# hengdashi/cuda_gcn

Measured on AMD Instinct MI355X. Metric: epochs_per_sec, higher is better.
Workload: dtype f32

## Files before the change

cuda_gcn_amd/csrc/class_bf16x3.h:

```cpp
#pragma once
#include "dense_kernels.h"
#include "bf16x3_split.h"

struct ClsB3 { bf16x8 h, m, l; };

__device__ __forceinline__ ClsB3 cls_planes(const float v[8]) {
    BxPlanes P;
#pragma unroll
    for (int i = 0; i < 4; i++) bx_split2(v[2 * i], v[2 * i + 1], P.w[0][i], P.w[1][i], P.w[2][i]);
    return ClsB3{bx_plane(P, 0), bx_plane(P, 1), bx_plane(P, 2)};
}
__device__ __forceinline__ void cls_mac(f32x16 &c, const ClsB3 &A, const ClsB3 &B) {
    c = MFMA_BF16(A.l, B.h, c);
    c = MFMA_BF16(A.m, B.m, c);
    c = MFMA_BF16(A.h, B.l, c);
    c = MFMA_BF16(A.m, B.h, c);
    c = MFMA_BF16(A.h, B.m, c);
    c = MFMA_BF16(A.h, B.h, c);
}
__device__ __forceinline__ ClsB3 cls_lds(const uint4 *img, int piece, int lane) {
    const uint4 h = img[(piece * 3 + 0) * 64 + lane], m = img[(piece * 3 + 1) * 64 + lane], l = img[(piece * 3 + 2) * 64 + lane];
    return ClsB3{__builtin_bit_cast(bf16x8, h), __builtin_bit_cast(bf16x8, m), __builtin_bit_cast(bf16x8, l)};
}
__device__ __forceinline__ void cls_lds_put(uint4 *img, int piece, int lane, const float v[8]) {
    BxPlanes P;
#pragma unroll
    for (int i = 0; i < 4; i++) bx_split2(v[2 * i], v[2 * i + 1], P.w[0][i], P.w[1][i], P.w[2][i]);
#pragma unroll
    for (int pl = 0; pl < 3; pl++) img[(piece * 3 + pl) * 64 + lane] = make_uint4(P.w[pl][0], P.w[pl][1], P.w[pl][2], P.w[pl][3]);
}

struct ClsFwdArgs {
    const float *h1; int ldh;
    const float *w2; int ldw;
    float *z0; int ldz;
    int m, p, n_rb;
};
constexpr int CLS_FWD_LDS = 8 * 2 * 3 * 1024;

#define CLS_WAIT2(N, x, y) asm volatile("s_waitcnt vmcnt(" #N ")" : "+v"(x), "+v"(y) :: "memory")
template <int S>
__device__ __forceinline__ void cls_fwd_issue(f32x4 (&R)[16], uint32_t vo, u32x4 rs) {
    bx_bload16<64 * S>(R[2 * S], vo, rs);
    bx_bload16<64 * S + 16>(R[2 * S + 1], vo, rs);
}

#define CLS_TIE4(R, i) "+v"((R)[i]), "+v"((R)[(i) + 1]), "+v"((R)[(i) + 2]), "+v"((R)[(i) + 3])
#define CLS_WAIT_ALL16(R) asm volatile("s_waitcnt vmcnt(0)" : CLS_TIE4(R, 0), CLS_TIE4(R, 4), CLS_TIE4(R, 8), CLS_TIE4(R, 12) :: "memory")

__global__ __launch_bounds__(256) void class_fwd_bf16x3_kernel(ClsFwdArgs a) {
    extern __shared__ __attribute__((aligned(16))) uint4 cls_img[];
    const int lane = threadIdx.x & 63, wave = threadIdx.x >> 6, li = lane & 31, hh = lane >> 5;
    for (int idx = threadIdx.x; idx < 8 * 2 * 64; idx += 256) {
        const int ln = idx & 63, cb = (idx >> 6) & 1, s = idx >> 7;
        const int c = 32 * cb + (ln & 31), k0 = 16 * s + 8 * (ln >> 5);
        const bool ok = c < a.p;
        const float *wp = a.w2 + (size_t)k0 * a.ldw + (ok ? c : 0);
        float v[8];
#pragma unroll
        for (int j = 0; j < 8; j++) v[j] = wp[(size_t)j * a.ldw];
#pragma unroll
        for (int j = 0; j < 8; j++) v[j] = ok ? v[j] : 0.f;
        cls_lds_put(cls_img, s * 2 + cb, ln, v);
    }
    __syncthreads();
    const u32x4 rs_h = bx_make_rsrc(a.h1, (uint32_t)a.m * (uint32_t)a.ldh * 4u);
    const int stride = gridDim.x * 4;
    int rb = blockIdx.x * 4 + wave;
    auto voff = [&](int b) { return ((uint32_t)(b * 32 + li) * (uint32_t)a.ldh + 8u * hh) * 4u; };
    auto issue = [&](f32x4 (&Q)[16], uint32_t vo) __attribute__((always_inline)) {
        cls_fwd_issue<0>(Q, vo, rs_h); cls_fwd_issue<1>(Q, vo, rs_h); cls_fwd_issue<2>(Q, vo, rs_h); cls_fwd_issue<3>(Q, vo, rs_h);
        cls_fwd_issue<4>(Q, vo, rs_h); cls_fwd_issue<5>(Q, vo, rs_h); cls_fwd_issue<6>(Q, vo, rs_h); cls_fwd_issue<7>(Q, vo, rs_h);
    };
    f32x4 R[16];
    issue(R, voff(rb));
    for (; rb < a.n_rb; rb += stride) {
        const uint32_t vn = voff(rb + stride);
        f32x16 acc[2];
#pragma unroll
        for (int cb = 0; cb < 2; cb++)
#pragma unroll
            for (int r = 0; r < 16; r++) acc[cb][r] = 0.f;
#define CLS_FWD_STEP(S)                                                                                                      \
        {                                                                                                                    \
            CLS_WAIT2(14, R[2 * S], R[2 * S + 1]);                                                                           \
            const float v[8] = {R[2 * S][0], R[2 * S][1], R[2 * S][2], R[2 * S][3], R[2 * S + 1][0], R[2 * S + 1][1], R[2 * S + 1][2], R[2 * S + 1][3]}; \
            ClsB3 A = cls_planes(v);                                                                                         \
            asm volatile("" : "+v"(A.h), "+v"(A.m), "+v"(A.l));                \
            cls_fwd_issue<S>(R, vn, rs_h);                                                                                   \
            cls_mac(acc[0], A, cls_lds(cls_img, S * 2, lane));                                                               \
            if (a.p > 32) cls_mac(acc[1], A, cls_lds(cls_img, S * 2 + 1, lane));                                             \
        }
        CLS_FWD_STEP(0) CLS_FWD_STEP(1) CLS_FWD_STEP(2) CLS_FWD_STEP(3) CLS_FWD_STEP(4) CLS_FWD_STEP(5) CLS_FWD_STEP(6) CLS_FWD_STEP(7)
#undef CLS_FWD_STEP
#pragma unroll
        for (int cb = 0; cb < 2; cb++)
#pragma unroll
            for (int r = 0; r < 16; r++) {
                const int orow = rb * 32 + (r & 3) + 8 * (r >> 2) + 4 * hh, c = 32 * cb + li;
                if (orow < a.m && c < a.p) a.z0[(size_t)orow * a.ldz + c] = acc[cb][r];
            }
    }
    CLS_WAIT_ALL16(R);
}

struct ClsBwdArgs {
    const float *dz; int lddz;
    const float *h1; int ldh;
    const float *w2; int ldw;
    float *da; int ldda;
    const uint32_t *bits;
    const float *rowscale; float scale;
    float *slab; int p_ld;
    int m, p, n_rb;
};
constexpr int CLS_BWD_PAIRS = 4;
constexpr int CLS_BWD_IMG = 4 * 4 * 3 * 1024;
constexpr int CLS_BWD_LDS = CLS_BWD_IMG + 128 * 64 * 4;

struct ClsCol { float z[2][8], h[2][8]; };
#define CLS_TIE8(x) "+v"((x)[0]), "+v"((x)[1]), "+v"((x)[2]), "+v"((x)[3]), "+v"((x)[4]), "+v"((x)[5]), "+v"((x)[6]), "+v"((x)[7])
#define CLS_WAIT_COL(N, c) asm volatile("s_waitcnt vmcnt(%32)" : CLS_TIE8((c).z[0]), CLS_TIE8((c).z[1]), CLS_TIE8((c).h[0]), CLS_TIE8((c).h[1]) : "n"(N) : "memory")

template <int NKS>
__global__ __launch_bounds__(512) void class_bwd_bf16x3_kernel(ClsBwdArgs a) {
    extern __shared__ __attribute__((aligned(16))) uint4 cls_img[];
    float *red = reinterpret_cast<float *>(cls_img) + CLS_BWD_IMG / 4;
    const int lane = threadIdx.x & 63, wave = threadIdx.x >> 6, li = lane & 31, hh = lane >> 5;
    const int pair = wave >> 1, half = wave & 1;
    for (int idx = threadIdx.x; idx < NKS * 4 * 64; idx += 512) {
        const int ln = idx & 63, fb = (idx >> 6) & 3, s = idx >> 8;
        const int f = 32 * fb + (ln & 31), c0 = 16 * s + 8 * (ln >> 5);
        float v[8];
#pragma unroll
        for (int j = 0; j < 8; j++) v[j] = a.w2[(size_t)f * a.ldw + min(c0 + j, a.p - 1)];
#pragma unroll
        for (int j = 0; j < 8; j++) v[j] = c0 + j < a.p ? v[j] : 0.f;
        cls_lds_put(cls_img, s * 4 + fb, ln, v);
    }
    for (int i = threadIdx.x; i < 128 * 64; i += 512) red[i] = 0.f;
    __syncthreads();

    const u32x4 rs_z = bx_make_rsrc(a.dz, (uint32_t)a.m * (uint32_t)a.lddz * 4u);
    const u32x4 rs_h = bx_make_rsrc(a.h1, (uint32_t)a.m * (uint32_t)a.ldh * 4u);
    const u32x4 rs_b = bx_make_rsrc(a.bits, (uint32_t)a.m * 16u);
    const u32x4 rs_s = bx_make_rsrc(a.rowscale ? a.rowscale : a.dz, a.rowscale ? (uint32_t)a.m * 4u : 0u);
    uint32_t so_z[8], so_h[8];
#pragma unroll
    for (int j = 0; j < 8; j++) { so_z[j] = (uint32_t)j * (uint32_t)a.lddz * 4u; so_h[j] = (uint32_t)j * (uint32_t)a.ldh * 4u; }

    f32x4 Z[2 * NKS];
    f32x4 KB;
    float RSC;
    auto issue_l1 = [&](int b) __attribute__((always_inline)) {
        const uint32_t row = (uint32_t)(b * 32 + li);
        const uint32_t vz = (row * (uint32_t)a.lddz + 8u * hh) * 4u;
        bx_bload16<0>(Z[0], vz, rs_z); bx_bload16<16>(Z[1], vz, rs_z);
        if constexpr (NKS > 1) { bx_bload16<64>(Z[2], vz, rs_z); bx_bload16<80>(Z[3], vz, rs_z); }
        if constexpr (NKS > 2) { bx_bload16<128>(Z[4], vz, rs_z); bx_bload16<144>(Z[5], vz, rs_z); }
        if constexpr (NKS > 3) { bx_bload16<192>(Z[6], vz, rs_z); bx_bload16<208>(Z[7], vz, rs_z); }
        bx_bload16<0>(KB, row * 16u, rs_b); bx_bload4(RSC, row * 4u, rs_s, 0u);
    };
    constexpr int NL1 = 2 * NKS + 2;
    ClsCol Cc;
    auto issue_col = [&](int b, int s2) __attribute__((always_inline)) {
        const uint32_t r0 = (uint32_t)(b * 32 + 16 * s2 + 8 * hh);
#pragma unroll
        for (int cb = 0; cb < 2; cb++) {
            const uint32_t c = 32u * cb + li;
            const uint32_t vo = c < (uint32_t)a.lddz ? (r0 * (uint32_t)a.lddz + c) * 4u : 0xFFFFF000u;
#pragma unroll
            for (int j = 0; j < 8; j++) bx_bload4(Cc.z[cb][j], vo, rs_z, so_z[j]);
        }
#pragma unroll
        for (int f2 = 0; f2 < 2; f2++) {
            const uint32_t vo = (r0 * (uint32_t)a.ldh + 32u * (2 * half + f2) + li) * 4u;
#pragma unroll
            for (int j = 0; j < 8; j++) bx_bload4(Cc.h[f2][j], vo, rs_h, so_h[j]);
        }
    };

    f32x16 dw[2][2];
#pragma unroll
    for (int f2 = 0; f2 < 2; f2++)
#pragma unroll
        for (int cb = 0; cb < 2; cb++)
#pragma unroll
            for (int r = 0; r < 16; r++) dw[f2][cb][r] = 0.f;

    const int stride = gridDim.x * CLS_BWD_PAIRS;
    int rb = blockIdx.x * CLS_BWD_PAIRS + pair;
    issue_l1(rb);
    for (; rb < a.n_rb; rb += stride) {
        issue_col(rb, 0);
        asm volatile("s_waitcnt vmcnt(32)" : "+v"(KB), "+v"(RSC) :: "memory");
#pragma unroll
        for (int i = 0; i < 2 * NKS; i++) asm volatile("" : "+v"(Z[i]));
        const uint32_t kw[2] = {__float_as_uint(KB[2 * half]), __float_as_uint(KB[2 * half + 1])};
        const float sc = a.rowscale ? a.scale * RSC : a.scale;
        f32x16 acc[2];
#pragma unroll
        for (int f2 = 0; f2 < 2; f2++)
#pragma unroll
            for (int r = 0; r < 16; r++) acc[f2][r] = 0.f;
#pragma unroll
        for (int s = 0; s < NKS; s++) {
            float v[8] = {Z[2 * s][0], Z[2 * s][1], Z[2 * s][2], Z[2 * s][3], Z[2 * s + 1][0], Z[2 * s + 1][1], Z[2 * s + 1][2], Z[2 * s + 1][3]};
            const int c0 = 16 * s + 8 * hh;
#pragma unroll
            for (int j = 0; j < 8; j++) v[j] = c0 + j < a.p ? v[j] : 0.f;
            const ClsB3 B = cls_planes(v);
#pragma unroll
            for (int f2 = 0; f2 < 2; f2++) cls_mac(acc[f2], B, cls_lds(cls_img, s * 4 + 2 * half + f2, lane));
        }
#pragma unroll
        for (int r = 0; r < 16; r++) {
            const int rl = (r & 3) + 8 * (r >> 2) + 4 * hh, orow = rb * 32 + rl;
            const float scr = __shfl(sc, rl, WAVE);
            const uint32_t w0 = __shfl(kw[0], rl, WAVE), w1 = __shfl(kw[1], rl, WAVE);
            if (orow < a.m) {
                float *dp = a.da + (size_t)orow * a.ldda + 64 * half + li;
                dp[0] = ((w0 >> li) & 1u) ? acc[0][r] * scr : 0.f;
                dp[32] = ((w1 >> li) & 1u) ? acc[1][r] * scr : 0.f;
            }
        }
        issue_l1(rb + stride);
#pragma unroll
        for (int s2 = 0; s2 < 2; s2++) {
            if (s2 == 0) CLS_WAIT_COL(NL1, Cc);
            else CLS_WAIT_COL(0, Cc);
            ClsB3 Bz[2], Ah[2];
#pragma unroll
            for (int cb = 0; cb < 2; cb++) {
                float v[8];
#pragma unroll
                for (int j = 0; j < 8; j++) v[j] = (32 * cb + li < a.p) ? Cc.z[cb][j] : 0.f;
                Bz[cb] = cls_planes(v);
            }
#pragma unroll
            for (int f2 = 0; f2 < 2; f2++) Ah[f2] = cls_planes(Cc.h[f2]);
            if (s2 == 0) issue_col(rb, 1);
#pragma unroll
            for (int f2 = 0; f2 < 2; f2++) {
                cls_mac(dw[f2][0], Ah[f2], Bz[0]);
                if (a.p > 32) cls_mac(dw[f2][1], Ah[f2], Bz[1]);
            }
        }
        asm volatile("s_waitcnt vmcnt(0)" : "+v"(KB), "+v"(RSC) :: "memory");
#pragma unroll
        for (int i = 0; i < 2 * NKS; i++) asm volatile("" : "+v"(Z[i]));
    }
    asm volatile("s_waitcnt vmcnt(0)" : "+v"(KB), "+v"(RSC) :: "memory");
#pragma unroll
    for (int i = 0; i < 2 * NKS; i++) asm volatile("" : "+v"(Z[i]));
    for (int w = 0; w < CLS_BWD_PAIRS; w++) {
        if (pair == w) {
#pragma unroll
            for (int f2 = 0; f2 < 2; f2++)
#pragma unroll
                for (int cb = 0; cb < 2; cb++)
#pragma unroll
                    for (int r = 0; r < 16; r++) {
                        const int f = 32 * (2 * half + f2) + (r & 3) + 8 * (r >> 2) + 4 * hh;
                        red[f * 64 + 32 * cb + li] += dw[f2][cb][r];
                    }
        }
        __syncthreads();
    }
    float *slab = a.slab + (size_t)blockIdx.x * 128 * a.p_ld;
    for (int i = threadIdx.x; i < 128 * a.p_ld; i += 512) {
        const int f = i / a.p_ld, c = i % a.p_ld;
        slab[i] = c < 64 ? red[f * 64 + c] : 0.f;
    }
}

static inline bool cls_fwd_fits(const float *a, int lda, const float *c, int ldc, int m, int n, int p) {
    return n == 128 && p >= 1 && p <= 64 && m >= 2048 && lda % 4 == 0 && lda >= 128 && ldc % 4 == 0 && aligned16(a) && aligned16(c) &&
           (uint64_t)m * lda * 4 < (1ull << 32);
}
static inline bool cls_bwd_fits(const float *a, int lda, const float *dc, int lddc, const float *da, int ldda, const uint32_t *bits, int wpr,
                                int m, int n, int p) {
    return n == 128 && p >= 1 && p <= 64 && m >= 2048 && wpr == 4 && bits && aligned16(bits) && a && lda >= 128 && lddc % 4 == 0 &&
           lddc >= (p + 15) / 16 * 16 && ldda % 4 == 0 && ldda >= 128 && aligned16(dc) && aligned16(da) &&
           (uint64_t)m * lda * 4 < (1ull << 32) && (uint64_t)m * lddc * 4 < (1ull << 32);
}

static int launch_class_fwd(gcnhip_ctx *c, const float *a, int lda, const float *b, int ldb, float *z, int ldz, int m, int p) {
    ClsFwdArgs k;
    k.h1 = a; k.ldh = lda; k.w2 = b; k.ldw = ldb; k.z0 = z; k.ldz = ldz; k.m = m; k.p = p; k.n_rb = ceil_div(m, 32);
    int grid = ceil_div(k.n_rb, 4);
    if (grid > c->n_cu * 3) grid = c->n_cu * 3;
    class_fwd_bf16x3_kernel<<<grid, 256, CLS_FWD_LDS, c->stream>>>(k);
    GCNHIP_LAUNCH_CHECK();
    return 0;
}
```

cuda_gcn_amd/csrc/matmul.hip:

```cpp
#include "dense_kernels.h"
#include "class_bf16x3.h"

extern "C" {

int gcnhip_matmul_fwd(gcnhip_ctx *c, const float *a, int lda, const float *b, int ldb,
                      float *cc, int ldc, int m, int n, int p) {
    if (!c || !a || !b || !cc || m < 0 || n <= 0 || p <= 0 || lda < n || ldb < p || ldc < p) return -1;
    if (m == 0) return 0;
    if (c->opt.gemm_bf16x3 >= 1 && cls_fwd_fits(a, lda, cc, ldc, m, n, p)) return launch_class_fwd(c, a, lda, b, ldb, cc, ldc, m, p);
    return launch_rowstream(c, a, lda, b, ldb, 0, cc, ldc, m, n, p, nullptr, 0, 1.f);
}

static int launch_class_bwd(gcnhip_ctx *c, const float *a, int lda, const float *b, int ldb, const float *dc, int lddc, float *da, int ldda,
                            float *db, int lddb, int m, int p, float scale, const uint32_t *bits, const float *rowscale) {
    ClsBwdArgs k;
    k.dz = dc; k.lddz = lddc; k.h1 = a; k.ldh = lda; k.w2 = b; k.ldw = ldb; k.da = da; k.ldda = ldda; k.bits = bits;
    k.rowscale = rowscale; k.scale = scale; k.p_ld = (p + 3) / 4 * 4; k.m = m; k.p = p; k.n_rb = ceil_div(m, 32);
    const int nks = (p + 15) / 16;
    int grid = ceil_div(k.n_rb, CLS_BWD_PAIRS);
    if (grid > c->n_cu) grid = c->n_cu;
    const int rc = ensure_slab(c, (size_t)grid * 128 * k.p_ld * sizeof(float));
    if (rc) return rc;
    k.slab = c->slab;
#define CLS_BWD(NKS)                                                                                                              \
    do {                                                                                                                          \
        GCNHIP_TRY(hipFuncSetAttribute((const void *)class_bwd_bf16x3_kernel<NKS>, hipFuncAttributeMaxDynamicSharedMemorySize, CLS_BWD_LDS)); \
        class_bwd_bf16x3_kernel<NKS><<<grid, 512, CLS_BWD_LDS, c->stream>>>(k);                                                  \
    } while (0)
    switch (nks) {
        case 1: CLS_BWD(1); break;
        case 2: CLS_BWD(2); break;
        case 3: CLS_BWD(3); break;
        default: CLS_BWD(4); break;
    }
#undef CLS_BWD
    GCNHIP_LAUNCH_CHECK();
    launch_slab_reduce(k.slab, grid, 128, p, k.p_ld, db, lddb, c->stream);
    GCNHIP_LAUNCH_CHECK();
    return 0;
}

static int da_product(gcnhip_ctx *c, bool fits_only, const float *dc, int lddc, const float *b, int ldb, float *da, int ldda, int m, int n, int p,
                      const float *h, int ldh, float scale, const uint32_t *bits, int wpr, const float *rowscale) {
    if (fits_only) return rowstream_plan(dc, lddc, da, ldda, p, n, h, ldh, bits).fits ? 0 : -1;
    return launch_rowstream(c, dc, lddc, b, ldb, 1, da, ldda, m, p, n, h, ldh, scale, bits, wpr, rowscale);
}

static int matmul_bwd_impl(gcnhip_ctx *c, const float *a, int lda, const float *b, int ldb,
                           const float *dc, int lddc, float *da, int ldda, float *db, int lddb,
                           int m, int n, int p, int fused, float scale) {
    if (!c || !a || !b || !dc || m < 0 || n <= 0 || p <= 0 || lda < n || ldb < p || lddc < p) return -1;
    if ((da && ldda < n) || (db && lddb < p)) return -1;
    if (m == 0) {
        if (db) for (int j = 0; j < n; j++) GCNHIP_TRY(hipMemsetAsync(db + (size_t)j * lddb, 0, p * sizeof(float), c->stream));
        return 0;
    }
    auto da_call = [&](bool fits_only) { return da_product(c, fits_only, dc, lddc, b, ldb, da, ldda, m, n, p, fused ? a : nullptr, lda, scale, nullptr, 0, nullptr); };
    if (da && da_call(true)) return -1;
    if (db) {
        const int rc = launch_atb(c, a, lda, dc, lddc, db, lddb, m, n, p, 0, 0.f, 0, nullptr, 0, nullptr);
        if (rc) return rc;
    }
    return da ? da_call(false) : 0;
}

int gcnhip_matmul_bwd(gcnhip_ctx *c, const float *a, int lda, const float *b, int ldb,
                      const float *dc, int lddc, float *da, int ldda, float *db, int lddb,
                      int m, int n, int p) {
    return matmul_bwd_impl(c, a, lda, b, ldb, dc, lddc, da, ldda, db, lddb, m, n, p, 0, 1.f);
}

int gcnhip_matmul_bwd_fused(gcnhip_ctx *c, const float *a, int lda, const float *b, int ldb,
                            const float *dc, int lddc, float *da, int ldda, float *db, int lddb,
                            int m, int n, int p, float relu_dropout_scale) {
    return matmul_bwd_impl(c, a, lda, b, ldb, dc, lddc, da, ldda, db, lddb, m, n, p, 1, relu_dropout_scale);
}

int gcnhip_matmul_bwd_fused_bits(gcnhip_ctx *c, const float *a, int lda, const float *b, int ldb,
                                 const float *dc, int lddc, float *da, int ldda, float *db, int lddb,
                                 int m, int n, int p, float relu_dropout_scale, const uint32_t *pos_bits, int words_per_row) {
    if (!c || !a || !b || !dc || !da || !pos_bits || m < 0 || n <= 0 || p <= 0 || lda < n || ldb < p || lddc < p || ldda < n) return -1;
    if (db && lddb < p) return -1;
    if (words_per_row * 32 < n) return -1;
    if (m == 0) return matmul_bwd_impl(c, a, lda, b, ldb, dc, lddc, nullptr, 0, db, lddb, m, n, p, 0, 1.f);
    auto da_call = [&](bool fits_only) {
        return da_product(c, fits_only, dc, lddc, b, ldb, da, ldda, m, n, p, nullptr, 0, relu_dropout_scale, pos_bits, words_per_row, nullptr);
    };
    if (da_call(true)) return -1;
    if (db) {
        const int rc = launch_atb(c, a, lda, dc, lddc, db, lddb, m, n, p, 0, 0.f, 0, nullptr, 0, nullptr);
        if (rc) return rc;
    }
    return da_call(false);
}

int gcnhip_matmul_bwd_ex(gcnhip_ctx *c, const float *a, int lda, const float *b, int ldb,
                         const float *dc, int lddc, float *da, int ldda, float *db, int lddb,
                         int m, int n, int p, float relu_dropout_scale, const uint32_t *pos_bits, int words_per_row,
                         const float *d_da_row_scale) {
    if (!c || !b || !dc || !da || m < 0 || n <= 0 || p <= 0 || ldb < p || lddc < p || ldda < n) return -1;
    if ((db || !pos_bits) && (!a || lda < n)) return -1;
    if (db && lddb < p) return -1;
    if (pos_bits && words_per_row * 32 < n) return -1;
    if (!(relu_dropout_scale > 0.f)) return -1;
    if (m == 0) {
        if (db) for (int j = 0; j < n; j++) GCNHIP_TRY(hipMemsetAsync(db + (size_t)j * lddb, 0, p * sizeof(float), c->stream));
        return 0;
    }
    if (db && c->opt.gemm_bf16x3 >= 1 && cls_bwd_fits(a, lda, dc, lddc, da, ldda, pos_bits, words_per_row, m, n, p))
        return launch_class_bwd(c, a, lda, b, ldb, dc, lddc, da, ldda, db, lddb, m, p, relu_dropout_scale, pos_bits, d_da_row_scale);
// ... 25 lines not shown
```

cuda_gcn_amd/csrc/graphsum.hip:

```cpp
#include "dense_kernels.h"
#include <algorithm>
#include <stdlib.h>

struct GsArgs {
    const int *indptr, *indices;
    const float *coef;
    const int4 *tasks;
    int n_tasks, n_rows, nnz;
    size_t table_bytes;
    const float *in;
    const uint16_t *in_bf;
    float *out;
    float *partials;
    int ld_in, ld_out, part_ld, dim;
    int n_slices;
    int bounds[9];
    int fuse, training, thr;
    float scale;
    uint64_t seed, elem_offset;
    const uint32_t *d_epoch;
    const uint8_t *keep_mask;
    const uint32_t *row_bits;
    const uint32_t *out_bits;
    uint32_t *pos_bits;
// ... 45 lines not shown
#pragma unroll
        for (int i = 0; i < 4; i++) x[i] *= (bits >> i & 1u) ? a.scale : 0.f;
    }
    return make_float4(x[0], x[1], x[2], x[3]);
}

template <int L>
__device__ __forceinline__ void xent_row_epilogue4(const GsArgs &a, int row, float4 z, int lane, int l, int g, int col0) {
#pragma clang fp contract(off)
    const int t = a.xe_truth[row];
    const int nv4 = (a.dim + 3) >> 2;
    float *gr = a.xe_grad ? a.xe_grad + (size_t)row * a.xe_ld_grad : nullptr;
    if (t < 0) {
        if (a.xe_training && gr && g == 0 && l < nv4) *reinterpret_cast<float4 *>(gr + col0) = make_float4(0.f, 0.f, 0.f, 0.f);
        if (lane == 0) *reinterpret_cast<float2 *>(a.xe_terms + 2 * (size_t)row) = make_float2(0.f, 0.f);
        return;
    }
    float x[4] = {z.x, z.y, z.z, z.w};
    float mx = -1e30f;
#pragma unroll
    for (int i = 0; i < 4; i++) if (col0 + i < a.dim) mx = fmaxf(mx, x[i]);
#pragma unroll
    for (int m = 1; m < L; m <<= 1) mx = fmaxf(mx, __shfl_xor(mx, m, WAVE));
    mx = __int_as_float(__builtin_amdgcn_readfirstlane(__float_as_int(mx)));
    const int ti = t & 3;
    const float sel = ti == 0 ? x[0] : (ti == 1 ? x[1] : (ti == 2 ? x[2] : x[3]));
    const float tv = __int_as_float(__builtin_amdgcn_readlane(__float_as_int(sel), t >> 2));
    const bool correct = !(mx > tv);
    float ex[4];
#pragma unroll
    for (int i = 0; i < 4; i++) {
        x[i] -= mx;
        ex[i] = col0 + i < a.dim ? expf(x[i]) : 0.f;
    }
    float se = 0.f;
    for (int q = 0; q < nv4; q++) {
#pragma unroll
        for (int i = 0; i < 4; i++) se += __int_as_float(__builtin_amdgcn_readlane(__float_as_int(ex[i]), q));
    }
    const float term = logf(se) - (tv - mx);
    if (lane == 0) *reinterpret_cast<float2 *>(a.xe_terms + 2 * (size_t)row) = make_float2(term, correct ? 1.f : 0.f);
    if (a.xe_training && gr && g == 0 && l < nv4) {
        const float gs = a.xe_grad_scale ? a.xe_grad_scale[row] : 1.f;
        float o[4];
#pragma unroll
        for (int i = 0; i < 4; i++) {
            float p = ex[i] / se;
            if (col0 + i == t) p = (float)((double)p - 1.0);
            o[i] = col0 + i < a.dim ? (a.xe_grad_scale ? (p / a.xe_count) * gs : p / a.xe_count) : 0.f;
        }
        *reinterpret_cast<float4 *>(gr + col0) = make_float4(o[0], o[1], o[2], o[3]);
    }
}
__device__ __forceinline__ void xent_row_epilogue1(const GsArgs &a, int row, float v, int lane) {
#pragma clang fp contract(off)
    const int t = a.xe_truth[row];
    const int nv4 = (a.dim + 3) >> 2;
    float *gr = a.xe_grad ? a.xe_grad + (size_t)row * a.xe_ld_grad : nullptr;
    if (t < 0) {
        if (a.xe_training && gr && lane < 4 * nv4) gr[lane] = 0.f;
        if (lane == 0) *reinterpret_cast<float2 *>(a.xe_terms + 2 * (size_t)row) = make_float2(0.f, 0.f);
        return;
    }
    float mx = lane < a.dim ? fmaxf(-1e30f, v) : -1e30f;
#pragma unroll
    for (int m = 1; m < WAVE; m <<= 1) mx = fmaxf(mx, __shfl_xor(mx, m, WAVE));
    const float tv = __int_as_float(__builtin_amdgcn_readlane(__float_as_int(v), t));
    const bool correct = !(mx > tv);
    const float x = v - mx;
    const float ex = lane < a.dim ? expf(x) : 0.f;
    float se = 0.f;
    for (int j = 0; j < 4 * nv4; j++) se += __int_as_float(__builtin_amdgcn_readlane(__float_as_int(ex), j));
    const float term = logf(se) - (tv - mx);
    if (lane == 0) *reinterpret_cast<float2 *>(a.xe_terms + 2 * (size_t)row) = make_float2(term, correct ? 1.f : 0.f);
    if (a.xe_training && gr && lane < 4 * nv4) {
        float p = ex / se;
        if (lane == t) p = (float)((double)p - 1.0);
        const float gs = a.xe_grad_scale ? a.xe_grad_scale[row] : 1.f;
        gr[lane] = lane < a.dim ? (a.xe_grad_scale ? (p / a.xe_count) * gs : p / a.xe_count) : 0.f;
    }
}

constexpr int GS_U = 4;
template <int L, int GS_U>
__device__ __forceinline__ float4 gather_chunk(const GsArgs &a, const float *in, int my_idx, float my_c, int cnt, int g, float4 acc) {
    constexpr int G = WAVE / L;
    const int iters = (cnt + G - 1) / G;
    int k = 0;
    if (!a.row_bits) {
        for (; (k + GS_U) * G <= cnt; k += GS_U) {
            float4 v[GS_U];
            float cc[GS_U];
#pragma unroll
            for (int u = 0; u < GS_U; u++) {
                const int src = (k + u) * G + g;
                const int j = __shfl(my_idx, src, WAVE);
                cc[u] = __shfl(my_c, src, WAVE);
                v[u] = *reinterpret_cast<const float4 *>(in + (size_t)j * a.ld_in);
            }
#pragma unroll
            for (int u = 0; u < GS_U; u++) acc = f4_fma(cc[u], v[u], acc);
        }
    }
    const int j_safe = __shfl(my_idx, 0, WAVE);
    for (; k < iters; k += GS_U) {
        float4 v[GS_U];
        float cc[GS_U];
        bool on[GS_U];
#pragma unroll
        for (int u = 0; u < GS_U; u++) {
            const int src = (k + u) * G + g;
            const int j = __shfl(my_idx, src & 63, WAVE);
            cc[u] = __shfl(my_c, src & 63, WAVE);
            on[u] = src < cnt && cc[u] != 0.f;
            v[u] = *reinterpret_cast<const float4 *>(in + (size_t)(on[u] ? j : j_safe) * a.ld_in);
        }
#pragma unroll
        for (int u = 0; u < GS_U; u++) {
            const float4 n = f4_fma(cc[u], v[u], acc);
            acc.x = on[u] ? n.x : acc.x; acc.y = on[u] ? n.y : acc.y; acc.z = on[u] ? n.z : acc.z; acc.w = on[u] ? n.w : acc.w;
        }
    }
    return acc;
}


struct GsTask { int row, e0, e1, slot; };
__device__ __forceinline__ GsTask gs_task(const GsArgs &a, int t) {
    if (a.n_tasks) {
        const int4 tk = a.tasks[t];
        return {tk.x, tk.y, tk.z, tk.w};
    }
    return {t, a.indptr[t], a.indptr[t + 1], -1};
}

template <bool SLICED>
__device__ __forceinline__ bool gs_block_task(const GsArgs &a, int &t, int &cslice) {
    const int xcd = blockIdx.x & 7, q = blockIdx.x >> 3;
    cslice = SLICED ? xcd % a.n_slices : blockIdx.y;
    const int g_id = SLICED ? xcd / a.n_slices : xcd;
    t = a.bounds[g_id] + q * (blockDim.x >> 6) + (threadIdx.x >> 6);
    return t < a.bounds[g_id + 1];
}

__device__ __forceinline__ void gs_load_edges(const GsArgs &a, int base, int cnt, int lane, int &my_idx, float &my_c) {
    my_idx = 0;
    my_c = 0.f;
    if (lane < cnt) {
        my_idx = a.indices[base + lane];
        my_c = a.coef ? a.coef[base + lane] : 1.f;
        if (a.row_bits && !((a.row_bits[my_idx >> 5] >> (my_idx & 31)) & 1u)) my_c = 0.f;
    }
}

template <int L>
__device__ __forceinline__ float4 gs_group_sum(float4 acc) {
#pragma unroll
    for (int m = L; m < WAVE; m <<= 1) acc = f4_add(acc, f4_shfl_xor(acc, m));
    return acc;
}

__device__ __forceinline__ void gs_store_partial(const GsArgs &a, int slot, int col0, float4 acc) {
    *reinterpret_cast<float4 *>(a.partials + (size_t)slot * a.part_ld + col0) = acc;
}
__device__ __forceinline__ void gs_store_partial(const GsArgs &a, int slot, int col0, float4 lo, float4 hi) {
    gs_store_partial(a, slot, col0, lo);
    gs_store_partial(a, slot, col0 + 4, hi);
}

__device__ __forceinline__ float gs_segment_sum(const GsArgs &a, int first, int ns, int col, float v) {
    const float *pp = a.partials + (size_t)first * a.part_ld + col;
    int k = 0;
    for (; k + 4 <= ns; k += 4) {
        const float p0 = pp[(size_t)k * a.part_ld], p1 = pp[(size_t)(k + 1) * a.part_ld];
        const float p2 = pp[(size_t)(k + 2) * a.part_ld], p3 = pp[(size_t)(k + 3) * a.part_ld];
        v += p0; v += p1; v += p2; v += p3;
    }
    const float p0 = pp[(size_t)min(k, ns - 1) * a.part_ld], p1 = pp[(size_t)min(k + 1, ns - 1) * a.part_ld];
    const float p2 = pp[(size_t)min(k + 2, ns - 1) * a.part_ld];
    if (k < ns) v += p0;
    if (k + 1 < ns) v += p1;
    if (k + 2 < ns) v += p2;
    return v;
}

__device__ __forceinline__ float4 gs_post4(const GsArgs &a, int row, float4 acc) {
    if (a.post) { const float ps = a.post[row]; acc.x *= ps; acc.y *= ps; acc.z *= ps; acc.w *= ps; }
    return acc;
}
__device__ __forceinline__ void gs_store_row4(const GsArgs &a, float *o, int col0, float4 acc) {
    if (col0 + 4 <= a.dim) {
        *reinterpret_cast<float4 *>(o) = acc;
    } else {
        const float x[4] = {acc.x, acc.y, acc.z, acc.w};
        for (int i = 0; col0 + i < a.dim; i++) o[i] = x[i];
    }
}

template <int L, int U = GS_U, bool SLICED = false>
__global__ __launch_bounds__(256) void graphsum_vec_kernel(GsArgs a) {
    const int lane = threadIdx.x & 63;
    int t, cslice;
    if (!gs_block_task<SLICED>(a, t, cslice)) return;
    const auto [row, e0, e1, slot] = gs_task(a, t);
    if (!row_wanted(a, row)) return;
    const int g = lane / L, l = lane % L;
    const int col0 = (cslice * L + l) * 4;
    const bool active = col0 < a.dim;
    const float *in = a.in + (active ? col0 : 0);
    float4 acc = make_float4(0.f, 0.f, 0.f, 0.f);
    for (int base = e0; base < e1; base += WAVE) {
        const int cnt = min(WAVE, e1 - base);
        int my_idx;
        float my_c;
        gs_load_edges(a, base, cnt, lane, my_idx, my_c);
        acc = gather_chunk<L, U>(a, in, my_idx, my_c, cnt, g, acc);
    }
    if constexpr (L < WAVE) acc = gs_group_sum<L>(acc);
    if (slot >= 0) {
        if (g == 0 && active) gs_store_partial(a, slot, col0, acc);
        return;
    }
    uint32_t nib = 0;
    if (g == 0 && active) {
        float *o = a.out + (size_t)row * a.ld_out + col0;
        if (a.accumulate && slot < 0) {
            if (col0 + 4 <= a.dim) {
                acc = f4_add(*reinterpret_cast<const float4 *>(o), acc);
            } else {
                float x[4] = {acc.x, acc.y, acc.z, acc.w};
                for (int i = 0; col0 + i < a.dim; i++) x[i] = o[i] + x[i];
                acc = make_float4(x[0], x[1], x[2], x[3]);
            }
        }
        acc = gs_post4(a, row, acc);
        if (a.fuse) acc = relu_dropout4(acc, a, row, col0);
        gs_store_row4(a, o, col0, acc);
        nib = ((acc.x > 0.f ? 1u : 0u) | (acc.y > 0.f ? 2u : 0u) | (acc.z > 0.f ? 4u : 0u) | (acc.w > 0.f ? 8u : 0u)) << (4 * (l & 7));
    }
    if constexpr (!SLICED && L <= 16)
        if (a.xe_truth) xent_row_epilogue4<L>(a, row, acc, lane, l, g, col0);
    if (L >= 8 && a.pos_bits) {
        nib |= __shfl_xor(nib, 1, WAVE);
        nib |= __shfl_xor(nib, 2, WAVE);
        nib |= __shfl_xor(nib, 4, WAVE);
        if (g == 0 && active && (l & 7) == 0) a.pos_bits[(size_t)row * a.wpr + (col0 >> 5)] = nib;
    }
}

__device__ inline void bf8_fma(float c, const uint4 v, float4 &lo, float4 &hi) {
    lo.x += c * __uint_as_float(v.x << 16); lo.y += c * __uint_as_float(v.x & 0xFFFF0000u);
    lo.z += c * __uint_as_float(v.y << 16); lo.w += c * __uint_as_float(v.y & 0xFFFF0000u);
    hi.x += c * __uint_as_float(v.z << 16); hi.y += c * __uint_as_float(v.z & 0xFFFF0000u);
    hi.z += c * __uint_as_float(v.w << 16); hi.w += c * __uint_as_float(v.w & 0xFFFF0000u);
}

template <int L>
__device__ __forceinline__ void gather_chunk_bf16(const GsArgs &a, const uint16_t *in, int my_idx, float my_c, int cnt, int g, float4 &lo, float4 &hi) {
    constexpr int G = WAVE / L;
    const int iters = (cnt + G - 1) / G;
    int k = 0;
    if (!a.row_bits) {
        for (; (k + GS_U) * G <= cnt; k += GS_U) {
            uint4 v[GS_U];
            float cc[GS_U];
#pragma unroll
            for (int u = 0; u < GS_U; u++) {
                const int src = (k + u) * G + g;
                const int j = __shfl(my_idx, src, WAVE);
                cc[u] = __shfl(my_c, src, WAVE);
                v[u] = *reinterpret_cast<const uint4 *>(in + (size_t)j * a.ld_in);
            }
#pragma unroll
            for (int u = 0; u < GS_U; u++) bf8_fma(cc[u], v[u], lo, hi);
        }
    }
    const int j_safe = __shfl(my_idx, 0, WAVE);
    for (; k < iters; k += GS_U) {
        uint4 v[GS_U];
        float cc[GS_U];
        bool on[GS_U];
#pragma unroll
        for (int u = 0; u < GS_U; u++) {
            const int src = (k + u) * G + g;
            const int j = __shfl(my_idx, src & 63, WAVE);
            cc[u] = __shfl(my_c, src & 63, WAVE);
            on[u] = src < cnt && cc[u] != 0.f;
            v[u] = *reinterpret_cast<const uint4 *>(in + (size_t)(on[u] ? j : j_safe) * a.ld_in);
        }
#pragma unroll
        for (int u = 0; u < GS_U; u++) {
            float4 nlo = lo, nhi = hi;
            bf8_fma(cc[u], v[u], nlo, nhi);
            lo.x = on[u] ? nlo.x : lo.x; lo.y = on[u] ? nlo.y : lo.y; lo.z = on[u] ? nlo.z : lo.z; lo.w = on[u] ? nlo.w : lo.w;
            hi.x = on[u] ? nhi.x : hi.x; hi.y = on[u] ? nhi.y : hi.y; hi.z = on[u] ? nhi.z : hi.z; hi.w = on[u] ? nhi.w : hi.w;
        }
    }
}
// ... 738 lines not shown
```

Baseline: 352.2.

## Warp-specialize classifier backward into dA and dW wave roles

Splits the backward classifier kernel's waves into two roles. One set of four waves computes the dA product over all 128 features per row block. The other four waves stream dz and h1 columns to accumulate the full dW, instead of each wave pair splitting features and doing both jobs. Row-block loads are now issued a full iteration ahead per role, and the forward kernel gains an unguarded fast-path store for full row blocks. This doubles the dW accumulator registers per wave and makes dA waves process twice the features, which risks register pressure and imbalance between the roles.

```diff
diff --git a/cuda_gcn_amd/csrc/class_bf16x3.h b/cuda_gcn_amd/csrc/class_bf16x3.h
--- a/cuda_gcn_amd/csrc/class_bf16x3.h
+++ b/cuda_gcn_amd/csrc/class_bf16x3.h
@@ -93,6 +93,15 @@
         }
         CLS_FWD_STEP(0) CLS_FWD_STEP(1) CLS_FWD_STEP(2) CLS_FWD_STEP(3) CLS_FWD_STEP(4) CLS_FWD_STEP(5) CLS_FWD_STEP(6) CLS_FWD_STEP(7)
 #undef CLS_FWD_STEP
+        if (rb * 32 + 32 <= a.m) {
+            float *zp = a.z0 + (size_t)(rb * 32 + 4 * hh) * a.ldz + li;
+#pragma unroll
+            for (int cb = 0; cb < 2; cb++)
+                if (32 * cb + li < a.p) {
+#pragma unroll
+                    for (int r = 0; r < 16; r++) zp[(size_t)((r & 3) + 8 * (r >> 2)) * a.ldz + 32 * cb] = acc[cb][r];
+                }
+        } else
 #pragma unroll
         for (int cb = 0; cb < 2; cb++)
 #pragma unroll
@@ -117,18 +126,21 @@
 constexpr int CLS_BWD_PAIRS = 4;
 constexpr int CLS_BWD_IMG = 4 * 4 * 3 * 1024;
 constexpr int CLS_BWD_LDS = CLS_BWD_IMG + 128 * 64 * 4;
-
-struct ClsCol { float z[2][8], h[2][8]; };
+constexpr int CLS_BWD_THREADS = 64 * 2 * CLS_BWD_PAIRS;
+
+struct ClsCol { float z[2][8], h[4][8]; };
 #define CLS_TIE8(x) "+v"((x)[0]), "+v"((x)[1]), "+v"((x)[2]), "+v"((x)[3]), "+v"((x)[4]), "+v"((x)[5]), "+v"((x)[6]), "+v"((x)[7])
-#define CLS_WAIT_COL(N, c) asm volatile("s_waitcnt vmcnt(%32)" : CLS_TIE8((c).z[0]), CLS_TIE8((c).z[1]), CLS_TIE8((c).h[0]), CLS_TIE8((c).h[1]) : "n"(N) : "memory")
+#define CLS_WAIT_Z(N, c) asm volatile("s_waitcnt vmcnt(%16)" : CLS_TIE8((c).z[0]), CLS_TIE8((c).z[1]) : "n"(N) : "memory")
+#define CLS_WAIT_H(N, c, f) asm volatile("s_waitcnt vmcnt(%8)" : CLS_TIE8((c).h[f]) : "n"(N) : "memory")
+#define CLS_PIN(P) asm volatile("" : "+v"((P).h), "+v"((P).m), "+v"((P).l))
 
 template <int NKS>
-__global__ __launch_bounds__(512) void class_bwd_bf16x3_kernel(ClsBwdArgs a) {
+__global__ __launch_bounds__(CLS_BWD_THREADS) void class_bwd_bf16x3_kernel(ClsBwdArgs a) {
     extern __shared__ __attribute__((aligned(16))) uint4 cls_img[];
     float *red = reinterpret_cast<float *>(cls_img) + CLS_BWD_IMG / 4;
-    const int lane = threadIdx.x & 63, wave = threadIdx.x >> 6, li = lane & 31, hh = lane >> 5;
-    const int pair = wave >> 1, half = wave & 1;
-    for (int idx = threadIdx.x; idx < NKS * 4 * 64; idx += 512) {
+    const int lane = threadIdx.x & 63, wave = __builtin_amdgcn_readfirstlane(threadIdx.x >> 6), li = lane & 31, hh = lane >> 5;
+    const int pair = wave & 3, role = wave >> 2;
+    for (int idx = threadIdx.x; idx < NKS * 4 * 64; idx += CLS_BWD_THREADS) {
         const int ln = idx & 63, fb = (idx >> 6) & 3, s = idx >> 8;
         const int f = 32 * fb + (ln & 31), c0 = 16 * s + 8 * (ln >> 5);
         float v[8];
@@ -138,137 +150,167 @@
         for (int j = 0; j < 8; j++) v[j] = c0 + j < a.p ? v[j] : 0.f;
         cls_lds_put(cls_img, s * 4 + fb, ln, v);
     }
-    for (int i = threadIdx.x; i < 128 * 64; i += 512) red[i] = 0.f;
+    for (int i = threadIdx.x; i < 128 * 64; i += CLS_BWD_THREADS) red[i] = 0.f;
     __syncthreads();
 
     const u32x4 rs_z = bx_make_rsrc(a.dz, (uint32_t)a.m * (uint32_t)a.lddz * 4u);
     const u32x4 rs_h = bx_make_rsrc(a.h1, (uint32_t)a.m * (uint32_t)a.ldh * 4u);
-    const u32x4 rs_b = bx_make_rsrc(a.bits, (uint32_t)a.m * 16u);
-    const u32x4 rs_s = bx_make_rsrc(a.rowscale ? a.rowscale : a.dz, a.rowscale ? (uint32_t)a.m * 4u : 0u);
-    uint32_t so_z[8], so_h[8];
-#pragma unroll
-    for (int j = 0; j < 8; j++) { so_z[j] = (uint32_t)j * (uint32_t)a.lddz * 4u; so_h[j] = (uint32_t)j * (uint32_t)a.ldh * 4u; }
-
-    f32x4 Z[2 * NKS];
-    f32x4 KB;
-    float RSC;
-    auto issue_l1 = [&](int b) __attribute__((always_inline)) {
-        const uint32_t row = (uint32_t)(b * 32 + li);
-        const uint32_t vz = (row * (uint32_t)a.lddz + 8u * hh) * 4u;
-        bx_bload16<0>(Z[0], vz, rs_z); bx_bload16<16>(Z[1], vz, rs_z);
-        if constexpr (NKS > 1) { bx_bload16<64>(Z[2], vz, rs_z); bx_bload16<80>(Z[3], vz, rs_z); }
-        if constexpr (NKS > 2) { bx_bload16<128>(Z[4], vz, rs_z); bx_bload16<144>(Z[5], vz, rs_z); }
-        if constexpr (NKS > 3) { bx_bload16<192>(Z[6], vz, rs_z); bx_bload16<208>(Z[7], vz, rs_z); }
-        bx_bload16<0>(KB, row * 16u, rs_b); bx_bload4(RSC, row * 4u, rs_s, 0u);
-    };
-    constexpr int NL1 = 2 * NKS + 2;
-    ClsCol Cc;
-    auto issue_col = [&](int b, int s2) __attribute__((always_inline)) {
-        const uint32_t r0 = (uint32_t)(b * 32 + 16 * s2 + 8 * hh);
-#pragma unroll
-        for (int cb = 0; cb < 2; cb++) {
-            const uint32_t c = 32u * cb + li;
-            const uint32_t vo = c < (uint32_t)a.lddz ? (r0 * (uint32_t)a.lddz + c) * 4u : 0xFFFFF000u;
-#pragma unroll
-            for (int j = 0; j < 8; j++) bx_bload4(Cc.z[cb][j], vo, rs_z, so_z[j]);
-        }
-#pragma unroll
-        for (int f2 = 0; f2 < 2; f2++) {
-            const uint32_t vo = (r0 * (uint32_t)a.ldh + 32u * (2 * half + f2) + li) * 4u;
-#pragma unroll
-            for (int j = 0; j < 8; j++) bx_bload4(Cc.h[f2][j], vo, rs_h, so_h[j]);
-        }
-    };
-
-    f32x16 dw[2][2];
-#pragma unroll
-    for (int f2 = 0; f2 < 2; f2++)
-#pragma unroll
-        for (int cb = 0; cb < 2; cb++)
-#pragma unroll
-            for (int r = 0; r < 16; r++) dw[f2][cb][r] = 0.f;
-
     const int stride = gridDim.x * CLS_BWD_PAIRS;
     int rb = blockIdx.x * CLS_BWD_PAIRS + pair;
-    issue_l1(rb);
-    for (; rb < a.n_rb; rb += stride) {
-        issue_col(rb, 0);
-        asm volatile("s_waitcnt vmcnt(32)" : "+v"(KB), "+v"(RSC) :: "memory");
-#pragma unroll
-        for (int i = 0; i < 2 * NKS; i++) asm volatile("" : "+v"(Z[i]));
-        const uint32_t kw[2] = {__float_as_uint(KB[2 * half]), __float_as_uint(KB[2 * half + 1])};
-        const float sc = a.rowscale ? a.scale * RSC : a.scale;
-        f32x16 acc[2];
-#pragma unroll
-        for (int f2 = 0; f2 < 2; f2++)
-#pragma unroll
-            for (int r = 0; r < 16; r++) acc[f2][r] = 0.f;
-#pragma unroll
-        for (int s = 0; s < NKS; s++) {
-            float v[8] = {Z[2 * s][0], Z[2 * s][1], Z[2 * s][2], Z[2 * s][3], Z[2 * s + 1][0], Z[2 * s + 1][1], Z[2 * s + 1][2], Z[2 * s + 1][3]};
-            const int c0 = 16 * s + 8 * hh;
-#pragma unroll
-            for (int j = 0; j < 8; j++) v[j] = c0 + j < a.p ? v[j] : 0.f;
-            const ClsB3 B = cls_planes(v);
-#pragma unroll
-            for (int f2 = 0; f2 < 2; f2++) cls_mac(acc[f2], B, cls_lds(cls_img, s * 4 + 2 * half + f2, lane));
+
+    f32x16 dw[4][2];
+#pragma unroll
+    for (int fb = 0; fb < 4; fb++)
+#pragma unroll
+        for (int cb = 0; cb < 2; cb++)
+#pragma unroll
+            for (int r = 0; r < 16; r++) dw[fb][cb][r] = 0.f;
+
+    if (role == 0) {
+        const u32x4 rs_b = bx_make_rsrc(a.bits, (uint32_t)a.m * 16u);
+        const u32x4 rs_s = bx_make_rsrc(a.rowscale ? a.rowscale : a.dz, a.rowscale ? (uint32_t)a.m * 4u : 0u);
+        f32x4 Z[2 * NKS];
+        f32x4 KB;
+        float RSC;
+        auto issue_l1 = [&](int b) __attribute__((always_inline)) {
+            const uint32_t row = (uint32_t)(b * 32 + li);
+            const uint32_t vz = (row * (uint32_t)a.lddz + 8u * hh) * 4u;
+            bx_bload16<0>(Z[0], vz, rs_z); bx_bload16<16>(Z[1], vz, rs_z);
+            if constexpr (NKS > 1) { bx_bload16<64>(Z[2], vz, rs_z); bx_bload16<80>(Z[3], vz, rs_z); }
+            if constexpr (NKS > 2) { bx_bload16<128>(Z[4], vz, rs_z); bx_bload16<144>(Z[5], vz, rs_z); }
+            if constexpr (NKS > 3) { bx_bload16<192>(Z[6], vz, rs_z); bx_bload16<208>(Z[7], vz, rs_z); }
+            bx_bload16<0>(KB, row * 16u, rs_b); bx_bload4(RSC, row * 4u, rs_s, 0u);
+        };
+        auto land_l1 = [&]() __attribute__((always_inline)) {
+            asm volatile("s_waitcnt vmcnt(0)" : "+v"(KB), "+v"(RSC) :: "memory");
+#pragma unroll
+            for (int i = 0; i < 2 * NKS; i++) asm volatile("" : "+v"(Z[i]));
+        };
+        issue_l1(rb);
+        land_l1();
+        for (; rb < a.n_rb; rb += stride) {
+            uint32_t kw[4] = {__float_as_uint(KB[0]), __float_as_uint(KB[1]), __float_as_uint(KB[2]), __float_as_uint(KB[3])};
+            float sc = a.rowscale ? a.scale * RSC : a.scale;
+            ClsB3 B[NKS];
+#pragma unroll
+            for (int s = 0; s < NKS; s++) {
+                float v[8] = {Z[2 * s][0], Z[2 * s][1], Z[2 * s][2], Z[2 * s][3], Z[2 * s + 1][0], Z[2 * s + 1][1], Z[2 * s + 1][2], Z[2 * s + 1][3]};
+                const int c0 = 16 * s + 8 * hh;
+#pragma unroll
+                for (int j = 0; j < 8; j++) v[j] = c0 + j < a.p ? v[j] : 0.f;
+                B[s] = cls_planes(v);
+                CLS_PIN(B[s]);
+            }
+            asm volatile("" : "+v"(kw[0]), "+v"(kw[1]), "+v"(kw[2]), "+v"(kw[3]), "+v"(sc));
+            issue_l1(rb + stride);
+#pragma unroll
+            for (int half = 0; half < 2; half++) {
+                float scr[16];
+                uint32_t w0[16], w1[16];
+#pragma unroll
+                for (int r = 0; r < 16; r++) {
+                    const int rl = (r & 3) + 8 * (r >> 2) + 4 * hh;
+                    scr[r] = __shfl(sc, rl, WAVE);
+                    w0[r] = __shfl(kw[2 * half], rl, WAVE);
+                    w1[r] = __shfl(kw[2 * half + 1], rl, WAVE);
+                }
+                f32x16 acc[2];
+#pragma unroll
+                for (int f2 = 0; f2 < 2; f2++)
+#pragma unroll
+                    for (int r = 0; r < 16; r++) acc[f2][r] = 0.f;
+#pragma unroll
+                for (int s = 0; s < NKS; s++)
+#pragma unroll
+                    for (int f2 = 0; f2 < 2; f2++) cls_mac(acc[f2], B[s], cls_lds(cls_img, s * 4 + 2 * half + f2, lane));
+                float *dp = a.da + (size_t)(rb * 32 + 4 * hh) * a.ldda + 64 * half + li;
+                if (rb * 32 + 32 <= a.m) {
+#pragma unroll
+                    for (int r = 0; r < 16; r++) {
+                        float *dr = dp + (size_t)((r & 3) + 8 * (r >> 2)) * a.ldda;
+                        dr[0] = ((w0[r] >> li) & 1u) ? acc[0][r] * scr[r] : 0.f;
+                        dr[32] = ((w1[r] >> li) & 1u) ? acc[1][r] * scr[r] : 0.f;
+                    }
+                } else {
+#pragma unroll
+                    for (int r = 0; r < 16; r++) {
+                        float *dr = dp + (size_t)((r & 3) + 8 * (r >> 2)) * a.ldda;
+                        if (rb * 32 + (r & 3) + 8 * (r >> 2) + 4 * hh < a.m) {
+                            dr[0] = ((w0[r] >> li) & 1u) ? acc[0][r] * scr[r] : 0.f;
+                            dr[32] = ((w1[r] >> li) & 1u) ? acc[1][r] * scr[r] : 0.f;
+                        }
+                    }
+                }
+            }
+            land_l1();
         }
-#pragma unroll
-        for (int r = 0; r < 16; r++) {
-            const int rl = (r & 3) + 8 * (r >> 2) + 4 * hh, orow = rb * 32 + rl;
-            const float scr = __shfl(sc, rl, WAVE);
-            const uint32_t w0 = __shfl(kw[0], rl, WAVE), w1 = __shfl(kw[1], rl, WAVE);
-            if (orow < a.m) {
-                float *dp = a.da + (size_t)orow * a.ldda + 64 * half + li;
-                dp[0] = ((w0 >> li) & 1u) ? acc[0][r] * scr : 0.f;
-                dp[32] = ((w1 >> li) & 1u) ? acc[1][r] * scr : 0.f;
+    } else {
+        uint32_t so_z[8], so_h[8];
+#pragma unroll
+        for (int j = 0; j < 8; j++) { so_z[j] = (uint32_t)j * (uint32_t)a.lddz * 4u; so_h[j] = (uint32_t)j * (uint32_t)a.ldh * 4u; }
+        ClsCol Cc;
+        auto row0 = [&](int b, int s2) { return (uint32_t)(b * 32 + 16 * s2 + 8 * hh); };
+        auto issue_z = [&](int b, int s2) __attribute__((always_inline)) {
+#pragma unroll
+            for (int cb = 0; cb < 2; cb++) {
+                const uint32_t c = 32u * cb + li;
+                const uint32_t vo = c < (uint32_t)a.lddz ? (row0(b, s2) * (uint32_t)a.lddz + c) * 4u : 0xFFFFF000u;
+#pragma unroll
+                for (int j = 0; j < 8; j++) bx_bload4(Cc.z[cb][j], vo, rs_z, so_z[j]);
+            }
+        };
+        auto issue_h = [&](int fb, int b, int s2) __attribute__((always_inline)) {
+            const uint32_t vo = (row0(b, s2) * (uint32_t)a.ldh + 32u * fb + li) * 4u;
+#pragma unroll
+            for (int j = 0; j < 8; j++) bx_bload4(Cc.h[fb][j], vo, rs_h, so_h[j]);
+        };
+        issue_z(rb, 0);
+#pragma unroll
+        for (int fb = 0; fb < 4; fb++) issue_h(fb, rb, 0);
+        for (; rb < a.n_rb; rb += stride) {
+#pragma unroll
+            for (int s2 = 0; s2 < 2; s2++) {
+                const int nb = s2 ? rb + stride : rb, ns = s2 ^ 1;
+                CLS_WAIT_Z(32, Cc);
+                ClsB3 Bz[2];
+#pragma unroll
+                for (int cb = 0; cb < 2; cb++) {
+                    float v[8];
+#pragma unroll
+                    for (int j = 0; j < 8; j++) v[j] = (32 * cb + li < a.p) ? Cc.z[cb][j] : 0.f;
+                    Bz[cb] = cls_planes(v);
+                    CLS_PIN(Bz[cb]);
+                }
+                issue_z(nb, ns);
+#pragma unroll
+                for (int fb = 0; fb < 4; fb++) {
+                    CLS_WAIT_H(40, Cc, fb);
+                    ClsB3 Ah = cls_planes(Cc.h[fb]);
+                    CLS_PIN(Ah);
+                    issue_h(fb, nb, ns);
+                    cls_mac(dw[fb][0], Ah, Bz[0]);
+                    if (a.p > 32) cls_mac(dw[fb][1], Ah, Bz[1]);
+                }
             }
         }
-        issue_l1(rb + stride);
-#pragma unroll
-        for (int s2 = 0; s2 < 2; s2++) {
-            if (s2 == 0) CLS_WAIT_COL(NL1, Cc);
-            else CLS_WAIT_COL(0, Cc);
-            ClsB3 Bz[2], Ah[2];
-#pragma unroll
-            for (int cb = 0; cb < 2; cb++) {
-                float v[8];
-#pragma unroll
-                for (int j = 0; j < 8; j++) v[j] = (32 * cb + li < a.p) ? Cc.z[cb][j] : 0.f;
-                Bz[cb] = cls_planes(v);
-            }
-#pragma unroll
-            for (int f2 = 0; f2 < 2; f2++) Ah[f2] = cls_planes(Cc.h[f2]);
-            if (s2 == 0) issue_col(rb, 1);
-#pragma unroll
-            for (int f2 = 0; f2 < 2; f2++) {
-                cls_mac(dw[f2][0], Ah[f2], Bz[0]);
-                if (a.p > 32) cls_mac(dw[f2][1], Ah[f2], Bz[1]);
-            }
-        }
-        asm volatile("s_waitcnt vmcnt(0)" : "+v"(KB), "+v"(RSC) :: "memory");
-#pragma unroll
-        for (int i = 0; i < 2 * NKS; i++) asm volatile("" : "+v"(Z[i]));
-    }
-    asm volatile("s_waitcnt vmcnt(0)" : "+v"(KB), "+v"(RSC) :: "memory");
-#pragma unroll
-    for (int i = 0; i < 2 * NKS; i++) asm volatile("" : "+v"(Z[i]));
+        asm volatile("s_waitcnt vmcnt(0)" : CLS_TIE8(Cc.z[0]), CLS_TIE8(Cc.z[1]), CLS_TIE8(Cc.h[0]), CLS_TIE8(Cc.h[1]), CLS_TIE8(Cc.h[2]), CLS_TIE8(Cc.h[3]) :: "memory");
+    }
     for (int w = 0; w < CLS_BWD_PAIRS; w++) {
-        if (pair == w) {
-#pragma unroll
-            for (int f2 = 0; f2 < 2; f2++)
+        if (role == 1 && pair == w) {
+#pragma unroll
+            for (int fb = 0; fb < 4; fb++)
 #pragma unroll
                 for (int cb = 0; cb < 2; cb++)
 #pragma unroll
                     for (int r = 0; r < 16; r++) {
-                        const int f = 32 * (2 * half + f2) + (r & 3) + 8 * (r >> 2) + 4 * hh;
-                        red[f * 64 + 32 * cb + li] += dw[f2][cb][r];
+                        const int f = 32 * fb + (r & 3) + 8 * (r >> 2) + 4 * hh;
+                        red[f * 64 + 32 * cb + li] += dw[fb][cb][r];
                     }
         }
         __syncthreads();
     }
     float *slab = a.slab + (size_t)blockIdx.x * 128 * a.p_ld;
-    for (int i = threadIdx.x; i < 128 * a.p_ld; i += 512) {
+    for (int i = threadIdx.x; i < 128 * a.p_ld; i += CLS_BWD_THREADS) {
         const int f = i / a.p_ld, c = i % a.p_ld;
         slab[i] = c < 64 ? red[f * 64 + c] : 0.f;
     }
diff --git a/cuda_gcn_amd/csrc/matmul.hip b/cuda_gcn_amd/csrc/matmul.hip
--- a/cuda_gcn_amd/csrc/matmul.hip
+++ b/cuda_gcn_amd/csrc/matmul.hip
@@ -25,7 +25,7 @@
 #define CLS_BWD(NKS)                                                                                                              \
     do {                                                                                                                          \
         GCNHIP_TRY(hipFuncSetAttribute((const void *)class_bwd_bf16x3_kernel<NKS>, hipFuncAttributeMaxDynamicSharedMemorySize, CLS_BWD_LDS)); \
-        class_bwd_bf16x3_kernel<NKS><<<grid, 512, CLS_BWD_LDS, c->stream>>>(k);                                                  \
+        class_bwd_bf16x3_kernel<NKS><<<grid, CLS_BWD_THREADS, CLS_BWD_LDS, c->stream>>>(k);                                                  \
     } while (0)
     switch (nks) {
         case 1: CLS_BWD(1); break;
```

After: 352.7 (median of 6 runs). Within noise of the previous version (+0.1%).

## Prefetch next edge chunk and specialize gather tail by remaining iterations

Applied to the files above, without the earlier changes.

The graphsum vector kernel now loads the next 64-edge chunk's indices and coefficients before gathering the current chunk, so the index loads overlap the feature gathers. The gather tail now dispatches to batch sizes 1 to 4 that match the remaining iterations, which avoids masked loads of unused slots. In the unmasked path only the last element of each tail batch is predicated. The cost is more register pressure and some extra code size from the instantiated variants.

```diff
diff --git a/cuda_gcn_amd/csrc/graphsum.hip b/cuda_gcn_amd/csrc/graphsum.hip
--- a/cuda_gcn_amd/csrc/graphsum.hip
+++ b/cuda_gcn_amd/csrc/graphsum.hip
@@ -151,8 +151,50 @@
 }
 
 constexpr int GS_U = 4;
+
+template <int L, int NB, bool MASKED>
+__device__ __forceinline__ float4 gather_batch(const GsArgs &a, const float *in, int my_idx, float my_c, int cnt, int k, int g, int j_safe, float4 acc) {
+    constexpr int G = WAVE / L;
+    float4 v[NB];
+    float cc[NB];
+    bool on[NB];
+#pragma unroll
+    for (int u = 0; u < NB; u++) {
+        const int src = (k + u) * G + g;
+        int j = __shfl(my_idx, src, WAVE);
+        cc[u] = __shfl(my_c, src, WAVE);
+        on[u] = true;
+        if (MASKED || u == NB - 1) {
+            on[u] = src < cnt && cc[u] != 0.f;
+            j = on[u] ? j : j_safe;
+        }
+        v[u] = *reinterpret_cast<const float4 *>(in + (size_t)j * a.ld_in);
+    }
+#pragma unroll
+    for (int u = 0; u < NB; u++) {
+        const float4 n = f4_fma(cc[u], v[u], acc);
+        if (MASKED || u == NB - 1) {
+            acc.x = on[u] ? n.x : acc.x; acc.y = on[u] ? n.y : acc.y; acc.z = on[u] ? n.z : acc.z; acc.w = on[u] ? n.w : acc.w;
+        } else {
+            acc = n;
+        }
+    }
+    return acc;
+}
+
+template <int L, int U, bool MASKED>
+__device__ __forceinline__ float4 gather_tail(const GsArgs &a, const float *in, int my_idx, float my_c, int cnt, int k, int nb, int g, int j_safe, float4 acc) {
+    switch (nb) {
+    case 4: if constexpr (U >= 4) return gather_batch<L, 4, MASKED>(a, in, my_idx, my_c, cnt, k, g, j_safe, acc); else break;
+    case 3: if constexpr (U >= 3) return gather_batch<L, 3, MASKED>(a, in, my_idx, my_c, cnt, k, g, j_safe, acc); else break;
+    case 2: if constexpr (U >= 2) return gather_batch<L, 2, MASKED>(a, in, my_idx, my_c, cnt, k, g, j_safe, acc); else break;
+    }
+    return gather_batch<L, 1, MASKED>(a, in, my_idx, my_c, cnt, k, g, j_safe, acc);
+}
+
 template <int L, int GS_U>
 __device__ __forceinline__ float4 gather_chunk(const GsArgs &a, const float *in, int my_idx, float my_c, int cnt, int g, float4 acc) {
+    static_assert(GS_U >= 1 && GS_U <= 4, "gather_tail dispatches on 1 .. 4 iterations");
     constexpr int G = WAVE / L;
     const int iters = (cnt + G - 1) / G;
     int k = 0;
@@ -170,26 +212,11 @@
 #pragma unroll
             for (int u = 0; u < GS_U; u++) acc = f4_fma(cc[u], v[u], acc);
         }
+        if (k < iters) acc = gather_tail<L, GS_U, false>(a, in, my_idx, my_c, cnt, k, iters - k, g, __shfl(my_idx, 0, WAVE), acc);
+        return acc;
     }
     const int j_safe = __shfl(my_idx, 0, WAVE);
-    for (; k < iters; k += GS_U) {
-        float4 v[GS_U];
-        float cc[GS_U];
-        bool on[GS_U];
-#pragma unroll
-        for (int u = 0; u < GS_U; u++) {
-            const int src = (k + u) * G + g;
-            const int j = __shfl(my_idx, src & 63, WAVE);
-            cc[u] = __shfl(my_c, src & 63, WAVE);
-            on[u] = src < cnt && cc[u] != 0.f;
-            v[u] = *reinterpret_cast<const float4 *>(in + (size_t)(on[u] ? j : j_safe) * a.ld_in);
-        }
-#pragma unroll
-        for (int u = 0; u < GS_U; u++) {
-            const float4 n = f4_fma(cc[u], v[u], acc);
-            acc.x = on[u] ? n.x : acc.x; acc.y = on[u] ? n.y : acc.y; acc.z = on[u] ? n.z : acc.z; acc.w = on[u] ? n.w : acc.w;
-        }
-    }
+    for (; k < iters; k += GS_U) acc = gather_tail<L, GS_U, true>(a, in, my_idx, my_c, cnt, k, min(GS_U, iters - k), g, j_safe, acc);
     return acc;
 }
 
@@ -278,11 +305,14 @@
     const bool active = col0 < a.dim;
     const float *in = a.in + (active ? col0 : 0);
     float4 acc = make_float4(0.f, 0.f, 0.f, 0.f);
+    int nx_idx = 0;
+    float nx_c = 0.f;
+    if (e0 < e1) gs_load_edges(a, e0, min(WAVE, e1 - e0), lane, nx_idx, nx_c);
     for (int base = e0; base < e1; base += WAVE) {
         const int cnt = min(WAVE, e1 - base);
-        int my_idx;
-        float my_c;
-        gs_load_edges(a, base, cnt, lane, my_idx, my_c);
+        const int my_idx = nx_idx;
+        const float my_c = nx_c;
+        if (base + WAVE < e1) gs_load_edges(a, base + WAVE, min(WAVE, e1 - base - WAVE), lane, nx_idx, nx_c);
         acc = gather_chunk<L, U>(a, in, my_idx, my_c, cnt, g, acc);
     }
     if constexpr (L < WAVE) acc = gs_group_sum<L>(acc);
```

New measurement: 347.5 before, 350.8 after (median of 6 runs). Within noise of the previous version (+0.9%).
